# dspcraft/dsc

Hardware: AMD Instinct MI355X
Metric: batched 1-D rfft GSamples/s (higher is better)
Workload: dtype f32

## Files before the change

dsc_amd/csrc/fft_c2c_32k.hip:

```cpp
#define DSC_R2C64K_HELPERS_ONLY 1
#include "fft_r2c_64k.hip"

namespace {

template<bool INV, bool CAST>
__global__ __launch_bounds__(1024) void c2c32k_kernel(const f2 *__restrict__ z, f2 *__restrict__ Z, int batch, const f2 *__restrict__ aux,
                                                      int in_pitch, int in_len) {
    constexpr int EB = CAST ? 4 : 8;
    auto sample = [](__amdgpu_buffer_rsrc_t r, int voff, int soff) {
        if constexpr (CAST) return cf{__builtin_bit_cast(float, __builtin_amdgcn_raw_buffer_load_b32(r, voff, soff, kStream)), 0.0f};
        else return load_c(r, voff, soff);
    };
    extern __shared__ __attribute__((aligned(16))) float lds[];
    float *plane = lds;
    f2 *T = (f2 *) (lds + kPlaneFloats);
    fill_twiddle_table(T, aux);
    const int wave_sgpr = __builtin_amdgcn_readfirstlane(threadIdx.x >> 6);
    constexpr float kScale = 1.0f / (float) kM;

    cf v[32];
    {
        const int row0 = blockIdx.x;
        const __amdgpu_buffer_rsrc_t r0 = __builtin_amdgcn_make_buffer_rsrc(
            (void *) ((const char *) z + (size_t) row0 * in_pitch * EB), 0, row0 < batch ? in_len * EB : 0, 0x00020000);
        const int load_off = thread_id(wave_sgpr) * EB;
#pragma unroll
        for (int a = 0; a < 32; ++a) v[a] = sample(r0, load_off, a * 1024 * EB);
    }
    for (int row = blockIdx.x; row < batch; row += gridDim.x) {
        const int next_row = row + gridDim.x;
        const __amdgpu_buffer_rsrc_t rnext = __builtin_amdgcn_make_buffer_rsrc(
            (void *) ((const char *) z + (size_t) next_row * in_pitch * EB), 0, next_row < batch ? in_len * EB : 0, 0x00020000);
        const __amdgpu_buffer_rsrc_t rout = __builtin_amdgcn_make_buffer_rsrc((void *) (Z + (size_t) row * kM), 0, kM * 8, 0x00020000);
        three_passes<INV>(v, plane, T, aux, wave_sgpr, false, false);
        if (INV) {
#pragma unroll
            for (int p = 0; p < 32; ++p) v[p] = cf{v[p].x * kScale, v[p].y * kScale};
        }
        const int load_off = thread_id(wave_sgpr) * EB;
        staged_time_store(v, plane, rout, wave_sgpr, [&](bool first_half) {
            if (first_half) {
#pragma unroll
                for (int a = 0; a < 16; ++a) v[2 * a] = sample(rnext, load_off, a * 1024 * EB);
            } else {
#pragma unroll
                for (int a = 16; a < 32; ++a) v[2 * (a - 16) + 1] = sample(rnext, load_off, a * 1024 * EB);
            }
        });
        unzip_rows(v);
    }
}

}

void dsc_launch_fft32k_c32(const void *z, void *Z, int batch, int in_pitch, int in_len, bool inverse, bool cast, const void *aux, int n_cu,
                           hipStream_t stream) {
    if (batch <= 0) return;
    static unsigned long long attr_devices = 0;
    if (dsc_first_use_on_device(attr_devices)) {
        DSC_KERNEL_CHECK(hipFuncSetAttribute((const void *) c2c32k_kernel<false, false>, hipFuncAttributeMaxDynamicSharedMemorySize, kLdsBytes));
        DSC_KERNEL_CHECK(hipFuncSetAttribute((const void *) c2c32k_kernel<true, false>, hipFuncAttributeMaxDynamicSharedMemorySize, kLdsBytes));
        DSC_KERNEL_CHECK(hipFuncSetAttribute((const void *) c2c32k_kernel<false, true>, hipFuncAttributeMaxDynamicSharedMemorySize, kLdsBytes));
        DSC_KERNEL_CHECK(hipFuncSetAttribute((const void *) c2c32k_kernel<true, true>, hipFuncAttributeMaxDynamicSharedMemorySize, kLdsBytes));
    }
    const int grid = batch < n_cu ? batch : n_cu;
#define C2C32K(INV, CAST) DSC_LAUNCH((c2c32k_kernel<INV, CAST>), dim3(grid), dim3(1024), kLdsBytes, stream, (const f2 *) z, (f2 *) Z, batch, (const f2 *) aux, in_pitch, in_len)
    if (inverse) { if (cast) C2C32K(true, true); else C2C32K(true, false); }
    else         { if (cast) C2C32K(false, true); else C2C32K(false, false); }
#undef C2C32K
}
```

dsc_amd/csrc/fft_r2c_64k.hip:

```cpp
#include "kernels.h"

#include <hip/hip_runtime.h>

#include <cmath>
#include <cstdlib>
#include <utility>

namespace {

typedef float f2 __attribute__((ext_vector_type(2)));

struct cf { float x, y; };
__device__ __forceinline__ cf operator+(cf a, cf b) { return cf{a.x + b.x, a.y + b.y}; }
__device__ __forceinline__ cf operator-(cf a, cf b) { return cf{a.x - b.x, a.y - b.y}; }
__device__ __forceinline__ cf to_cf(f2 a) { return cf{a.x, a.y}; }
__device__ __forceinline__ f2 to_f2(cf a) { return f2{a.x, a.y}; }

constexpr int kM = 32768;
constexpr int kRowPitch = 34;
constexpr int kPlaneFloats = 1024 * kRowPitch;
constexpr int kLdsBytes = kPlaneFloats * 4 + 1024 * 8;
constexpr int kTabEntries = 1024;

constexpr int kAuxW1024 = 0, kAuxW32768 = 1024, kAuxW65536 = 2048, kAuxEntries = 3072;

__host__ __device__ constexpr int br5(int x) {
    return ((x & 1) << 4) | ((x & 2) << 2) | (x & 4) | ((x & 8) >> 2) | ((x & 16) >> 4);
}

__device__ constexpr float kCos64[17] = {
    1.0f, 0.99518472667219688624f, 0.98078528040323044913f, 0.95694033573220886494f,
    0.92387953251128675613f, 0.88192126434835502971f, 0.83146961230254523708f, 0.77301045336273696081f,
    0.70710678118654752440f, 0.63439328416364549822f, 0.55557023301960222474f, 0.47139673682599764856f,
    0.38268343236508977173f, 0.29028467725446236764f, 0.19509032201612826785f, 0.09801714032956060199f,
    0.0f};

__device__ constexpr float root64_re(int q) {
    q &= 63;
    return q <= 16 ? kCos64[q] : q <= 32 ? -kCos64[32 - q] : q <= 48 ? -kCos64[q - 32] : kCos64[64 - q];
}
__device__ constexpr float root64_im(int q) {
    q &= 63;
    return q <= 16 ? -kCos64[16 - q] : q <= 32 ? -kCos64[q - 16] : q <= 48 ? kCos64[48 - q] : kCos64[q - 48];
}

__device__ __forceinline__ cf cmul(cf a, cf w) {
    return cf{a.x * w.x - a.y * w.y, a.x * w.y + a.y * w.x};
}
__device__ __forceinline__ cf cmul_conj(cf a, cf w) {
    return cf{a.x * w.x + a.y * w.y, a.y * w.x - a.x * w.y};
}

template<bool INV, int M, int K>
__device__ __forceinline__ cf mul_root(cf d) {
    constexpr float c8 = 0.70710678118654752440f;
    if constexpr (K == 0) {
        return d;
    } else if constexpr (4 * K == M) {
        return INV ? cf{-d.y, d.x} : cf{d.y, -d.x};
    } else if constexpr (8 * K == M) {
        return INV ? cf{(d.x - d.y) * c8, (d.x + d.y) * c8} : cf{(d.x + d.y) * c8, (d.y - d.x) * c8};
    } else if constexpr (8 * K == 3 * M) {
        return INV ? cf{-(d.x + d.y) * c8, (d.x - d.y) * c8} : cf{(d.y - d.x) * c8, -(d.x + d.y) * c8};
    } else {
        constexpr float wr = root64_re(K * (64 / M));
        constexpr float wi = INV ? -root64_im(K * (64 / M)) : root64_im(K * (64 / M));
        return cf{d.x * wr - d.y * wi, d.x * wi + d.y * wr};
    }
}

#ifdef DSC_DFT32_DIF
template<bool INV, int M, int G, int... K>
__device__ __forceinline__ void dif_group(cf (&v)[32], std::integer_sequence<int, K...>) {
    (([&] {
         const cf u = v[G + K] + v[G + K + M / 2];
         const cf d = v[G + K] - v[G + K + M / 2];
         v[G + K] = u;
         v[G + K + M / 2] = mul_root<INV, M, K>(d);
     }()),
     ...);
}

template<bool INV, int M, int... G>
__device__ __forceinline__ void dif_stage(cf (&v)[32], std::integer_sequence<int, G...>) {
    (dif_group<INV, M, G * M>(v, std::make_integer_sequence<int, M / 2>{}), ...);
}

template<bool INV>
__device__ __forceinline__ void dft32(cf (&v)[32]) {
    dif_stage<INV, 32>(v, std::make_integer_sequence<int, 1>{});
    dif_stage<INV, 16>(v, std::make_integer_sequence<int, 2>{});
    dif_stage<INV, 8>(v, std::make_integer_sequence<int, 4>{});
    dif_stage<INV, 4>(v, std::make_integer_sequence<int, 8>{});
    dif_stage<INV, 2>(v, std::make_integer_sequence<int, 16>{});
}


#else
constexpr double kCos64d[17] = {
    1.0, 0.99518472667219688624, 0.98078528040323044913, 0.95694033573220886494,
    0.92387953251128675613, 0.88192126434835502971, 0.83146961230254523708, 0.77301045336273696081,
    0.70710678118654752440, 0.63439328416364549822, 0.55557023301960222474, 0.47139673682599764856,
    0.38268343236508977173, 0.29028467725446236764, 0.19509032201612826785, 0.09801714032956060199,
    0.0};

template<bool INV, int E>
__device__ __forceinline__ void dit_butterfly(cf &a, cf &b) {
    if constexpr (E == 0) {
        const cf u = a + b, d = a - b;
        a = u; b = d;
    } else if constexpr (E == 8) {
        const cf u = INV ? cf{a.x - b.y, a.y + b.x} : cf{a.x + b.y, a.y - b.x};
        const cf d = INV ? cf{a.x + b.y, a.y - b.x} : cf{a.x - b.y, a.y + b.x};
        a = u; b = d;
    } else {
        constexpr double c = E <= 8 ? kCos64d[2 * E] : -kCos64d[32 - 2 * E];
        constexpr double sn = (E <= 8 ? kCos64d[16 - 2 * E] : kCos64d[2 * E - 16]);
        constexpr double s = INV ? sn : -sn;
        if constexpr ((c < 0 ? -c : c) >= sn) {
            constexpr float t = (float) (s / c), cc = (float) c;
            float p, q;
            if constexpr (t == 1.0f) { p = b.x - b.y; q = b.y + b.x; }
            else if constexpr (t == -1.0f) { p = b.x + b.y; q = b.y - b.x; }
            else { p = __builtin_fmaf(-t, b.y, b.x); q = __builtin_fmaf(t, b.x, b.y); }
            const cf u = cf{__builtin_fmaf(cc, p, a.x), __builtin_fmaf(cc, q, a.y)};
            const cf d = cf{__builtin_fmaf(-cc, p, a.x), __builtin_fmaf(-cc, q, a.y)};
            a = u; b = d;
        } else {
            constexpr float r = (float) (c / s), ss = (float) s;
            const float pn = __builtin_fmaf(-r, b.x, b.y);
            const float q = __builtin_fmaf(r, b.y, b.x);
            const cf u = cf{__builtin_fmaf(-ss, pn, a.x), __builtin_fmaf(ss, q, a.y)};
            const cf d = cf{__builtin_fmaf(ss, pn, a.x), __builtin_fmaf(-ss, q, a.y)};
            a = u; b = d;
        }
    }
}

constexpr int brev_bits(int x, int bits) {
    int r = 0;
    for (int i = 0; i < bits; ++i) r |= ((x >> i) & 1) << (bits - 1 - i);
    return r;
}

template<bool INV, int S, int G, int... J>
__device__ __forceinline__ void dit_group(cf (&v)[32], std::integer_sequence<int, J...>) {
    constexpr int H = 32 >> S;
    constexpr int E = brev_bits(G, S - 1) * (16 >> (S - 1));
    (dit_butterfly<INV, E>(v[2 * H * G + J], v[2 * H * G + J + H]), ...);
}

template<bool INV, int S, int... G>
__device__ __forceinline__ void dit_stage(cf (&v)[32], std::integer_sequence<int, G...>) {
    (dit_group<INV, S, G>(v, std::make_integer_sequence<int, (32 >> S)>{}), ...);
}

template<bool INV>
__device__ __forceinline__ void dft32(cf (&v)[32]) {
    dit_stage<INV, 1>(v, std::make_integer_sequence<int, 1>{});
    dit_stage<INV, 2>(v, std::make_integer_sequence<int, 2>{});
    dit_stage<INV, 3>(v, std::make_integer_sequence<int, 4>{});
    dit_stage<INV, 4>(v, std::make_integer_sequence<int, 8>{});
    dit_stage<INV, 5>(v, std::make_integer_sequence<int, 16>{});
}
#endif

typedef unsigned int u2 __attribute__((ext_vector_type(2)));
typedef unsigned int u4 __attribute__((ext_vector_type(4)));
typedef float f4 __attribute__((ext_vector_type(4)));

template<int COMP>
__device__ __forceinline__ void plane_write(float *plane, int wbase, const cf (&v)[32]) {
    int wbase_hi = wbase + 16 * (32 * kRowPitch);
    asm("" : "+v"(wbase_hi));
    float *lo16 = plane + wbase;
    float *hi16 = plane + wbase_hi;
#pragma unroll
    for (int p = 0; p < 32; p += 2) lo16[br5(p) * (32 * kRowPitch)] = COMP == 0 ? v[p].x : v[p].y;
#pragma unroll
    for (int p = 1; p < 32; p += 2) hi16[(br5(p) - 16) * (32 * kRowPitch)] = COMP == 0 ? v[p].x : v[p].y;
}

#ifndef DSC_LDS_SPLIT_READS
#define DSC_LDS_SPLIT_READS 1
#endif
__device__ __forceinline__ f2 lds_read_b64(const f2 *p) {
#if DSC_LDS_SPLIT_READS
    return *(const volatile __attribute__((address_space(3))) f2 *) p;
#else
    return *p;
#endif
}

template<int COMP>
__device__ __forceinline__ void plane_read(const float *plane, int row, cf (&v)[32]) {
    const f2 *r = (const f2 *) (plane + __mul24(row, kRowPitch));
#pragma unroll
    for (int m = 0; m < 16; ++m) {
        const f2 t = lds_read_b64(r + m);
        if (COMP == 0) { v[2 * m].x = t.x; v[2 * m + 1].x = t.y; }
        else           { v[2 * m].y = t.x; v[2 * m + 1].y = t.y; }
    }
}

__device__ __forceinline__ void lds_barrier() {
    __builtin_amdgcn_fence(__ATOMIC_RELEASE, "workgroup", "local");
    __builtin_amdgcn_s_barrier();
    __builtin_amdgcn_fence(__ATOMIC_ACQUIRE, "workgroup", "local");
}

__device__ __forceinline__ float bperm(int byte_addr, float x) {
    return __int_as_float(__builtin_amdgcn_ds_bpermute(byte_addr, __float_as_int(x)));
}

__device__ __forceinline__ int column_of(int wave, int lane) {
    int kp = lane < 32 ? 32 * wave + lane : 1024 - 32 * wave - (63 - lane);
    return kp == 1024 ? 512 : kp;
}

#ifdef DSC_R2C64K_PROBE
#define PROBE_ARGS , int io_on
#define PROBE_NULL , 1
#define IO_ON io_on
#else
#define PROBE_ARGS
#define PROBE_NULL
#define IO_ON 1
#endif

__device__ __forceinline__ int thread_id(int wave_sgpr) {
    int zero;
    asm volatile("v_mov_b32 %0, 0" : "=v"(zero));
    const int lane = __builtin_amdgcn_mbcnt_hi(-1, __builtin_amdgcn_mbcnt_lo(-1, zero));
    return (wave_sgpr << 6) | lane;
}

#ifndef DSC_STREAM_AUX
#define DSC_STREAM_AUX 2
#endif
constexpr int kStream = DSC_STREAM_AUX;
__device__ __forceinline__ cf load_c(__amdgpu_buffer_rsrc_t r, int voff, int soff) {
    return to_cf(__builtin_bit_cast(f2, __builtin_amdgcn_raw_buffer_load_b64(r, voff, soff, kStream)));
}
#ifndef DSC_FILTER_EARLY_LOADS
#define DSC_FILTER_EARLY_LOADS 4
#endif
#ifndef DSC_IRFFT_PIN_PASS3
#define DSC_IRFFT_PIN_PASS3 1
#endif
#ifndef DSC_IRFFT_EARLY_PAIRS
#define DSC_IRFFT_EARLY_PAIRS 4
#endif
#ifndef DSC_IRFFT_LOAD_AUX
#define DSC_IRFFT_LOAD_AUX 0
#endif
__device__ __forceinline__ cf load_c_spec(__amdgpu_buffer_rsrc_t r, int voff, int soff) {
    return to_cf(__builtin_bit_cast(f2, __builtin_amdgcn_raw_buffer_load_b64(r, voff, soff, DSC_IRFFT_LOAD_AUX)));
}
__device__ __forceinline__ cf load_c_cached(__amdgpu_buffer_rsrc_t r, int voff, int soff) {
    return to_cf(__builtin_bit_cast(f2, __builtin_amdgcn_raw_buffer_load_b64(r, voff, soff, 0)));
}
template<int POLICY>
__device__ __forceinline__ void store_c(cf a, __amdgpu_buffer_rsrc_t r, int voff, int soff) {
    __builtin_amdgcn_raw_buffer_store_b64(__builtin_bit_cast(u2, to_f2(a)), r, voff, soff, POLICY);
}

__device__ __forceinline__ void fill_twiddle_table(f2 *T, const f2 *aux) {
    const int t = threadIdx.x;
    T[t] = aux[kAuxW1024 + (t >> 5) * (t & 31)];
    __syncthreads();
}

__device__ __forceinline__ void exchange(float *plane, int wbase, int row, const cf (&src)[32], cf (&dst)[32]) {
    plane_write<0>(plane, wbase, src);
    lds_barrier();
    plane_read<0>(plane, row, dst);
    lds_barrier();
    plane_write<1>(plane, wbase, src);
    lds_barrier();
    plane_read<1>(plane, row, dst);
    lds_barrier();
}

struct no_hook { __device__ __forceinline__ void operator()() const {} };

template<bool INV, typename Hook = no_hook>
__device__ __forceinline__ void three_passes(cf (&v)[32], float *plane, const f2 *T, const f2 *aux, int wave_sgpr,
                                             bool mirrored_in, bool mirrored_out, Hook before_pass3 = Hook{}) {
    dft32<INV>(v);
    cf u[32];
    {
        const int t = thread_id(wave_sgpr);
        const int col = mirrored_in ? column_of(t >> 6, t & 63) : t;
        const int hi = col >> 5;
        const f2 *th = T + hi;
#pragma unroll
        for (int r1 = 1; r1 < 32; ++r1) {
            const cf w = to_cf(th[32 * r1]);
            v[br5(r1)] = INV ? cmul_conj(v[br5(r1)], w) : cmul(v[br5(r1)], w);
        }
        exchange(plane, __mul24(col & 31, kRowPitch) + hi, t, v, u);
    }
    dft32<INV>(u);
    {
        const int t = thread_id(wave_sgpr);
        const int hi = t >> 5, lo = t & 31;
        const cf tw2_base = to_cf(aux[kAuxW32768 + __mul24(hi, lo)]);
        u[0] = INV ? cmul_conj(u[0], tw2_base) : cmul(u[0], tw2_base);
        const f2 *tl = T + lo;
#pragma unroll
        for (int r2 = 1; r2 < 32; ++r2) {
            const cf w = cmul(tw2_base, to_cf(tl[32 * r2]));
            u[br5(r2)] = INV ? cmul_conj(u[br5(r2)], w) : cmul(u[br5(r2)], w);
        }
        const int col_out = mirrored_out ? column_of(t >> 6, t & 63) : t;
        exchange(plane, __mul24(hi, kRowPitch) + lo, col_out, u, v);
    }
    before_pass3();
    dft32<INV>(v);
}

__device__ __forceinline__ void real_pair(cf p, cf q, cf wq, float hs, cf &out_k, cf &out_mk) {
    const cf s = cf{p.x + q.x, p.y - q.y};
    const cf d = cf{p.x - q.x, p.y + q.y};
    const cf wd = cmul(d, wq);
    out_k = cf{hs * s.x + wd.x, hs * s.y + wd.y};
    out_mk = cf{hs * s.x - wd.x, wd.y - hs * s.y};
}

__device__ __forceinline__ int partner_byte_addr(int wave, int lane) {
    return ((wave == 0 && (lane == 63 || lane == 0)) ? lane : 63 - lane) * 4;
}

#ifndef DSC_R2C64K_HELPERS_ONLY
__global__ __launch_bounds__(1024) void rfft64k_kernel(const float *__restrict__ x, f2 *__restrict__ X, int batch,
                                                       const f2 *__restrict__ aux, int in_pitch, int in_len PROBE_ARGS) {
    extern __shared__ __attribute__((aligned(16))) float lds[];
    float *plane = lds;
    f2 *T = (f2 *) (lds + kPlaneFloats);
    fill_twiddle_table(T, aux);

    const int wave_sgpr = __builtin_amdgcn_readfirstlane(threadIdx.x >> 6);

    cf v[32];
    {
        const int row0 = blockIdx.x;
        const __amdgpu_buffer_rsrc_t r0 = __builtin_amdgcn_make_buffer_rsrc(
            (void *) (x + (size_t) row0 * in_pitch), 0, row0 < batch ? in_len * 4 * IO_ON : 0, 0x00020000);
        const int load_off = thread_id(wave_sgpr) * 8;
#pragma unroll
        for (int j1 = 0; j1 < 32; ++j1) v[j1] = load_c(r0, load_off, j1 * 8192);
    }

    for (int row = blockIdx.x; row < batch; row += gridDim.x) {
        const int next_row = row + gridDim.x;
        const __amdgpu_buffer_rsrc_t rnext = __builtin_amdgcn_make_buffer_rsrc(
            (void *) (x + (size_t) next_row * in_pitch), 0, next_row < batch ? in_len * 4 * IO_ON : 0, 0x00020000);
        const __amdgpu_buffer_rsrc_t rout =
            __builtin_amdgcn_make_buffer_rsrc((void *) (X + (size_t) row * (kM + 1)), 0, (kM + 1) * 8 * IO_ON, 0x00020000);

        three_passes<false>(v, plane, T, aux, wave_sgpr, false, true);

        const int t4 = thread_id(wave_sgpr);
        const int lane = t4 & 63, wave = t4 >> 6;
        const int kp = column_of(wave, lane);
        const int partner_addr = partner_byte_addr(wave, lane);
        cf xk[16], xm[16];
        const cf zmid = v[br5(16)];
        if (wave_sgpr == 0) {
#pragma unroll
            for (int r = 16; r < 31; ++r) v[br5(r)] = lane == 0 ? v[br5(r + 1)] : v[br5(r)];
            v[br5(31)] = lane == 0 ? v[br5(0)] : v[br5(31)];
        }
#pragma unroll
        for (int k3 = 0; k3 < 16; ++k3) {
            const int src = 31 - br5(k3);
            xm[k3].x = bperm(partner_addr, v[src].x);
            xm[k3].y = bperm(partner_addr, v[src].y);
        }
        {
            const cf wpost = to_cf(aux[kAuxW65536 + kp]);
            const cf post_base = cf{0.5f * wpost.y, -0.5f * wpost.x};
#pragma unroll
            for (int k3 = 0; k3 < 16; ++k3) {
                const cf c = cf{root64_re(k3), root64_im(k3)};
                const cf w = k3 == 0 ? post_base : cmul(post_base, c);
                real_pair(v[br5(k3)], xm[k3], w, 0.5f, xk[k3], xm[k3]);
            }
        }

        f2 *stage = (f2 *) plane;
        const int skew = (int) ((((size_t) (X + (size_t) row * (kM + 1))) >> 3) & 15);
#pragma unroll
        for (int k3 = 0; k3 < 16; ++k3) stage[kp + 1024 * k3] = to_f2(xk[k3]);
        const cf xk15 = xk[15];
        const int load_off = thread_id(wave_sgpr) * 8;
#pragma unroll
        for (int j1 = 0; j1 < 16; ++j1) v[j1] = load_c(rnext, load_off, j1 * 8192);
        lds_barrier();
#pragma unroll
        for (int m = 0; m < 8; ++m) {
            const int k = 2 * (t4 + 1024 * m) - skew;
            if (m > 0 || k >= 0) {
                const f2 lo2 = lds_read_b64(stage + k), hi2 = lds_read_b64(stage + k + 1);
                const f4 q = f4{lo2.x, lo2.y, hi2.x, hi2.y};
                __builtin_amdgcn_raw_buffer_store_b128(__builtin_bit_cast(u4, q), rout, k * 8, 0, kStream);
            } else if (m == 0 && k == -1) {
                __builtin_amdgcn_raw_buffer_store_b64(__builtin_bit_cast(u2, stage[0]), rout, 0, 0, kStream);
            }
            if (m & 1) __builtin_amdgcn_sched_barrier(0);
        }
        lds_barrier();
        constexpr int kStage2 = kM / 2 - 16;
#pragma unroll
        for (int k3 = 0; k3 < 16; ++k3) stage[(kM - kStage2) - kp - 1024 * k3] = to_f2(xm[k3]);
        if (kp >= 1009) stage[kp + 15 * 1024 - kStage2] = to_f2(xk15);
        if (t4 == 0) stage[kM / 2 - kStage2] = f2{zmid.x, -zmid.y};
#pragma unroll
        for (int j1 = 16; j1 < 32; ++j1) v[j1] = load_c(rnext, load_off, j1 * 8192);
        lds_barrier();
#pragma unroll
        for (int m = 0; m < 9; ++m) {
            if (m == 8 && wave != 0) break;
            const int k = kM / 2 + 2 * (t4 + 1024 * m) - skew;
            if (m < 8 || k + 1 <= kM) {
                const f2 lo2 = lds_read_b64(stage + k - kStage2), hi2 = lds_read_b64(stage + k + 1 - kStage2);
                const f4 q = f4{lo2.x, lo2.y, hi2.x, hi2.y};
                __builtin_amdgcn_raw_buffer_store_b128(__builtin_bit_cast(u4, q), rout, k * 8, 0, kStream);
            } else if (m == 8 && k == kM) {
                __builtin_amdgcn_raw_buffer_store_b64(__builtin_bit_cast(u2, stage[k - kStage2]), rout, k * 8, 0, kStream);
            }
            if (m & 1) __builtin_amdgcn_sched_barrier(0);
        }
        lds_barrier();
    }
}

#endif

__device__ __forceinline__ void inverse_prepass_direct(cf (&v)[32], cf y_mid, const f2 *aux, int wave_sgpr) {
    constexpr float kScale = 1.0f / (float) kM;
    const int t1 = thread_id(wave_sgpr);
    const int lane = t1 & 63, wave = t1 >> 6;
    const int c = column_of(wave, lane);
    const int partner_addr = partner_byte_addr(wave, lane);
    if (wave == 0 && lane == 0) { v[0].y = 0.f; v[16].y = 0.f; }
    const cf wpre = to_cf(aux[kAuxW65536 + c]);
    const cf wq_base = cf{0.5f * kScale * wpre.y, 0.5f * kScale * wpre.x};
#pragma unroll
    for (int half = 0; half < 2; ++half) {
        cf zm[8];
#pragma unroll
        for (int i = 0; i < 8; ++i) {
            const int a = half * 8 + i;
            const cf cj = cf{root64_re(a), -root64_im(a)};
            const cf wq = a == 0 ? wq_base : cmul(wq_base, cj);
            real_pair(v[a], v[16 + a], wq, 0.5f * kScale, v[a], zm[i]);
        }
#pragma unroll
        for (int i = 0; i < 8; ++i) {
            const int a = half * 8 + i;
            v[16 + a].x = bperm(partner_addr, zm[i].x);
            v[16 + a].y = bperm(partner_addr, zm[i].y);
        }
    }
    cf w[32];
#pragma unroll
    for (int r = 0; r < 16; ++r) { w[r] = v[r]; w[16 + r] = v[31 - r]; }
    if (wave == 0) {
#pragma unroll
        for (int r = 31; r > 16; --r) w[r] = lane == 0 ? w[r - 1] : w[r];
        w[16] = lane == 0 ? cf{kScale * y_mid.x, -kScale * y_mid.y} : w[16];
    }
#pragma unroll
    for (int r = 0; r < 32; ++r) v[r] = w[r];
}

template<typename IssueNext>
__device__ __forceinline__ void staged_time_store(cf (&v)[32], float *plane, __amdgpu_buffer_rsrc_t rout, int wave_sgpr,
                                                  IssueNext issue_next) {
    f2 *stage = (f2 *) plane;
    const int t4 = thread_id(wave_sgpr);
#pragma unroll
    for (int p = 0; p < 32; p += 2) stage[t4 + 1024 * br5(p)] = to_f2(v[p]);
    issue_next(true);
    lds_barrier();
#pragma unroll
    for (int m = 0; m < 8; ++m) {
        const int k = 2 * (t4 + 1024 * m);
        const f2 lo2 = lds_read_b64(stage + k), hi2 = lds_read_b64(stage + k + 1);
        const f4 q = f4{lo2.x, lo2.y, hi2.x, hi2.y};
        __builtin_amdgcn_raw_buffer_store_b128(__builtin_bit_cast(u4, q), rout, k * 8, 0, kStream);
        if (m & 1) __builtin_amdgcn_sched_barrier(0);
    }
    lds_barrier();
#pragma unroll
    for (int p = 1; p < 32; p += 2) stage[t4 + 1024 * (br5(p) - 16)] = to_f2(v[p]);
    issue_next(false);
    lds_barrier();
#pragma unroll
    for (int m = 0; m < 8; ++m) {
        const int k = 2 * (t4 + 1024 * m);
        const f2 lo2 = lds_read_b64(stage + k), hi2 = lds_read_b64(stage + k + 1);
        const f4 q = f4{lo2.x, lo2.y, hi2.x, hi2.y};
        __builtin_amdgcn_raw_buffer_store_b128(__builtin_bit_cast(u4, q), rout, (kM / 2 + k) * 8, 0, kStream);
        if (m & 1) __builtin_amdgcn_sched_barrier(0);
    }
    lds_barrier();
}

__device__ __forceinline__ void unzip_rows(cf (&v)[32]) {
    cf nxt[32];
#pragma unroll
    for (int a = 0; a < 16; ++a) { nxt[a] = v[2 * a]; nxt[16 + a] = v[2 * a + 1]; }
#pragma unroll
    for (int a = 0; a < 32; ++a) v[a] = nxt[a];
}

#ifndef DSC_R2C64K_HELPERS_ONLY
__global__ __launch_bounds__(1024) void irfft64k_kernel(const f2 *__restrict__ X, float *__restrict__ x, int batch,
                                                        const f2 *__restrict__ aux, int in_pitch, int in_len PROBE_ARGS) {
    extern __shared__ __attribute__((aligned(16))) float lds[];
    float *plane = lds;
    f2 *T = (f2 *) (lds + kPlaneFloats);
    fill_twiddle_table(T, aux);

    const int wave_sgpr = __builtin_amdgcn_readfirstlane(threadIdx.x >> 6);

    cf v[32];
    cf y_mid = cf{0.f, 0.f};
    {
        const int row0 = blockIdx.x;
        const __amdgpu_buffer_rsrc_t r0 = __builtin_amdgcn_make_buffer_rsrc(
            (void *) (X + (size_t) row0 * in_pitch), 0, row0 < batch ? in_len * 8 * IO_ON : 0, 0x00020000);
        const int t0 = thread_id(wave_sgpr);
        const int c = column_of(t0 >> 6, t0 & 63);
        const int pv = (kM - c - 15 * 1024) * 8;
#pragma unroll
        for (int a = 0; a < 16; ++a) {
            v[a] = load_c_spec(r0, c * 8, a * 8192);
            v[16 + a] = load_c_spec(r0, pv, (15 - a) * 8192);
        }
        if (c == 0) y_mid = load_c_spec(r0, (kM / 2) * 8, 0);
    }

    for (int row = blockIdx.x; row < batch; row += gridDim.x) {
        const int next_row = row + gridDim.x;
        const __amdgpu_buffer_rsrc_t rnext = __builtin_amdgcn_make_buffer_rsrc(
            (void *) (X + (size_t) next_row * in_pitch), 0, next_row < batch ? in_len * 8 * IO_ON : 0, 0x00020000);
        const __amdgpu_buffer_rsrc_t rout =
            __builtin_amdgcn_make_buffer_rsrc((void *) (x + (size_t) row * 65536), 0, 65536 * 4 * IO_ON, 0x00020000);

        inverse_prepass_direct(v, y_mid, aux, wave_sgpr);
        constexpr int kEarly = DSC_IRFFT_EARLY_PAIRS;
        cf early[kEarly > 0 ? 2 * kEarly : 1];
        three_passes<true>(v, plane, T, aux, wave_sgpr, true, false, [&]() {
            if constexpr (kEarly > 0) {
                const int t3 = thread_id(wave_sgpr);
                const int c3 = column_of(t3 >> 6, t3 & 63);
                const int pv3 = (kM - c3 - 15 * 1024) * 8;
#pragma unroll
                for (int a = 0; a < kEarly; ++a) {
                    early[2 * a] = load_c_spec(rnext, c3 * 8, a * 8192);
                    early[2 * a + 1] = load_c_spec(rnext, pv3, (15 - a) * 8192);
                }
            }
        });

#if DSC_IRFFT_PIN_PASS3
#pragma unroll
        for (int p = 0; p < 32; p += 8)
            asm volatile("" : "+v"(v[p].x), "+v"(v[p].y), "+v"(v[p + 1].x), "+v"(v[p + 1].y), "+v"(v[p + 2].x), "+v"(v[p + 2].y), "+v"(v[p + 3].x),
                         "+v"(v[p + 3].y), "+v"(v[p + 4].x), "+v"(v[p + 4].y), "+v"(v[p + 5].x), "+v"(v[p + 5].y), "+v"(v[p + 6].x), "+v"(v[p + 6].y),
                         "+v"(v[p + 7].x), "+v"(v[p + 7].y));
#endif
        const int t4 = thread_id(wave_sgpr);
        const int c = column_of(t4 >> 6, t4 & 63);
        const int pv = (kM - c - 15 * 1024) * 8;
        staged_time_store(v, plane, rout, wave_sgpr, [&](bool first_half) {
            if (first_half) {
                y_mid = cf{0.f, 0.f};
                if (c == 0) y_mid = load_c_spec(rnext, (kM / 2) * 8, 0);
#pragma unroll
                for (int i = 0; i < 8; ++i) {
                    v[2 * i] = load_c_spec(rnext, c * 8, (kEarly + i) * 8192);
                    v[16 + 2 * i] = load_c_spec(rnext, pv, (15 - kEarly - i) * 8192);
                }
            } else {
#pragma unroll
                for (int i = 0; i < 8 - kEarly; ++i) {
                    v[2 * i + 1] = load_c_spec(rnext, c * 8, (kEarly + 8 + i) * 8192);
                    v[17 + 2 * i] = load_c_spec(rnext, pv, (7 - kEarly - i) * 8192);
                }
            }
        });
        {
            cf nxt[32];
#pragma unroll
            for (int a = 0; a < 16; ++a) {
                if (a < kEarly)          { nxt[a] = early[2 * a];             nxt[16 + a] = early[2 * a + 1]; }
                else if (a < kEarly + 8) { nxt[a] = v[2 * (a - kEarly)];      nxt[16 + a] = v[16 + 2 * (a - kEarly)]; }
                else                     { nxt[a] = v[2 * (a - kEarly - 8) + 1]; nxt[16 + a] = v[17 + 2 * (a - kEarly - 8)]; }
            }
#pragma unroll
            for (int a = 0; a < 32; ++a) v[a] = nxt[a];
        }
    }
}

__global__ __launch_bounds__(1024) void filter64k_kernel(const float *__restrict__ x, const f2 *__restrict__ H,
                                                         float *__restrict__ y, int batch, const f2 *__restrict__ aux, int in_pitch,
                                                         int in_len) {
    extern __shared__ __attribute__((aligned(16))) float lds[];
    float *plane = lds;
    f2 *T = (f2 *) (lds + kPlaneFloats);
    fill_twiddle_table(T, aux);

    const int wave_sgpr = __builtin_amdgcn_readfirstlane(threadIdx.x >> 6);
    const __amdgpu_buffer_rsrc_t rh = __builtin_amdgcn_make_buffer_rsrc((void *) H, 0, (kM + 1) * 8, 0x00020000);
    constexpr float kScale = 1.0f / (float) kM;

    cf v[32];
    {
        const int row0 = blockIdx.x;
        const __amdgpu_buffer_rsrc_t r0 = __builtin_amdgcn_make_buffer_rsrc(
            (void *) (x + (size_t) row0 * in_pitch), 0, row0 < batch ? in_len * 4 : 0, 0x00020000);
        const int load_off = thread_id(wave_sgpr) * 8;
#pragma unroll
        for (int j1 = 0; j1 < 32; ++j1) v[j1] = load_c(r0, load_off, j1 * 8192);
    }
    for (int row = blockIdx.x; row < batch; row += gridDim.x) {
        const int next_row = row + gridDim.x;
        const __amdgpu_buffer_rsrc_t rnext = __builtin_amdgcn_make_buffer_rsrc(
            (void *) (x + (size_t) next_row * in_pitch), 0, next_row < batch ? in_len * 4 : 0, 0x00020000);
        const __amdgpu_buffer_rsrc_t rout =
            __builtin_amdgcn_make_buffer_rsrc((void *) (y + (size_t) row * 65536), 0, 65536 * 4, 0x00020000);
        three_passes<false>(v, plane, T, aux, wave_sgpr, false, true);

        {
            const int t1 = thread_id(wave_sgpr);
            const int lane = t1 & 63, wave = t1 >> 6;
            const int c = column_of(wave, lane);
            const int partner_addr = partner_byte_addr(wave, lane);
            const cf wc = to_cf(aux[kAuxW65536 + c]);
            const cf post_base = cf{0.5f * wc.y, -0.5f * wc.x};
            const cf pre_base = cf{0.5f * kScale * wc.y, 0.5f * kScale * wc.x};
            if (wave == 0) {
                const cf zmid = v[br5(16)];
                const cf hmid = load_c_cached(rh, (kM / 2) * 8, 0);
                const cf pmid = cmul(cf{zmid.x, -zmid.y}, hmid);
                v[br5(16)] = lane == 0 ? cf{kScale * pmid.x, -kScale * pmid.y} : v[br5(16)];
            }
            cf park = v[br5(16)];
            if (wave == 0) {
#pragma unroll
                for (int r = 16; r < 31; ++r) v[br5(r)] = lane == 0 ? v[br5(r + 1)] : v[br5(r)];
                v[br5(31)] = lane == 0 ? v[br5(0)] : v[br5(31)];
            }
#pragma unroll
            for (int part = 0; part < 8; ++part) {
                cf q[2], zm[2];
#pragma unroll
                for (int i = 0; i < 2; ++i) {
                    const int a = part * 2 + i;
                    q[i].x = bperm(partner_addr, v[br5(31 - a)].x);
                    q[i].y = bperm(partner_addr, v[br5(31 - a)].y);
                }
#pragma unroll
                for (int i = 0; i < 2; ++i) {
                    const int a = part * 2 + i;
                    const cf w64 = cf{root64_re(a), root64_im(a)};
                    cf xk, xm;
                    real_pair(v[br5(a)], q[i], a == 0 ? post_base : cmul(post_base, w64), 0.5f, xk, xm);
                    const cf hk = load_c_cached(rh, c * 8, a * 8192);
                    const cf hm = load_c_cached(rh, (kM - 15 * 1024 - c) * 8, (15 - a) * 8192);
                    cf pk = cmul(xk, hk), pm = cmul(xm, hm);
                    if (a == 0) {
                        pk.y = (c == 0) ? 0.f : pk.y;
                        pm.y = (c == 0) ? 0.f : pm.y;
                    }
                    const cf w64c = cf{root64_re(a), -root64_im(a)};
                    real_pair(pk, pm, a == 0 ? pre_base : cmul(pre_base, w64c), 0.5f * kScale, v[br5(a)], zm[i]);
                }
#pragma unroll
                for (int i = 0; i < 2; ++i) {
                    const int a = part * 2 + i;
                    v[br5(31 - a)].x = bperm(partner_addr, zm[i].x);
                    v[br5(31 - a)].y = bperm(partner_addr, zm[i].y);
                }
                __builtin_amdgcn_sched_barrier(0);
            }
            if (wave == 0) {
#pragma unroll
                for (int r = 31; r > 16; --r) v[br5(r)] = lane == 0 ? v[br5(r - 1)] : v[br5(r)];
                v[br5(16)] = lane == 0 ? park : v[br5(16)];
            }
        }
        cf z[32];
#pragma unroll
        for (int r = 0; r < 32; ++r) z[r] = v[br5(r)];
        constexpr int kEarlyX = DSC_FILTER_EARLY_LOADS;
        cf early[kEarlyX > 0 ? kEarlyX : 1];
        three_passes<true>(z, plane, T, aux, wave_sgpr, true, false, [&]() {
            if constexpr (kEarlyX > 0) {
                const int off = thread_id(wave_sgpr) * 8;
#pragma unroll
                for (int j1 = 0; j1 < kEarlyX; ++j1) early[j1] = load_c(rnext, off, j1 * 8192);
            }
        });
        {
            const int load_off = thread_id(wave_sgpr) * 8;
            staged_time_store(z, plane, rout, wave_sgpr, [&](bool first_half) {
                if (first_half) {
#pragma unroll
                    for (int i = 0; i < 16; ++i) z[2 * i] = load_c(rnext, load_off, (kEarlyX + i) * 8192);
                } else {
#pragma unroll
                    for (int i = 0; i < 16 - kEarlyX; ++i) z[2 * i + 1] = load_c(rnext, load_off, (kEarlyX + 16 + i) * 8192);
                }
            });
#pragma unroll
            for (int j1 = 0; j1 < 32; ++j1) v[j1] = j1 < kEarlyX ? early[j1] : j1 < kEarlyX + 16 ? z[2 * (j1 - kEarlyX)] : z[2 * (j1 - kEarlyX - 16) + 1];
        }
    }
}

#endif

}

#ifndef DSC_R2C64K_HELPERS_ONLY
size_t dsc_r2c64k_table_bytes() { return (size_t) kAuxEntries * sizeof(float) * 2; }

void dsc_r2c64k_build_tables(void *host_dst) {
    float *o = (float *) host_dst;
    auto put = [&](int at, long long k, long long n) {
        const long double a = -2.0L * 3.14159265358979323846264338327950288L * (long double) k / (long double) n;
        o[2 * at] = (float) cosl(a);
        o[2 * at + 1] = (float) sinl(a);
    };
    for (int m = 0; m < kTabEntries; ++m) {
        put(kAuxW1024 + m, m, 1024);
        put(kAuxW32768 + m, m, 32768);
        put(kAuxW65536 + m, m, 65536);
    }
    o[2 * (kAuxW1024 + 256)] = 0.f;  o[2 * (kAuxW1024 + 256) + 1] = -1.f;
    o[2 * (kAuxW1024 + 512)] = -1.f; o[2 * (kAuxW1024 + 512) + 1] = 0.f;
    o[2 * (kAuxW1024 + 768)] = 0.f;  o[2 * (kAuxW1024 + 768) + 1] = 1.f;
}

void dsc_launch_rfft64k(const float *x, void *X, int batch, int in_pitch, int in_len, const void *aux, int n_cu, hipStream_t stream) {
    if (batch <= 0) return;
    static unsigned long long attr_devices = 0;
    if (dsc_first_use_on_device(attr_devices)) {
        DSC_KERNEL_CHECK(hipFuncSetAttribute((const void *) rfft64k_kernel, hipFuncAttributeMaxDynamicSharedMemorySize, kLdsBytes));
    }
    const int grid = batch < n_cu ? batch : n_cu;
    DSC_LAUNCH(rfft64k_kernel, dim3(grid), dim3(1024), kLdsBytes, stream, x, (f2 *) X, batch, (const f2 *) aux, in_pitch, in_len PROBE_NULL);
}

void dsc_launch_irfft64k(const void *X, float *x, int batch, int in_pitch, int in_len, const void *aux, int n_cu, hipStream_t stream) {
    if (batch <= 0) return;
    static unsigned long long attr_devices = 0;
    if (dsc_first_use_on_device(attr_devices)) {
        DSC_KERNEL_CHECK(hipFuncSetAttribute((const void *) irfft64k_kernel, hipFuncAttributeMaxDynamicSharedMemorySize, kLdsBytes));
    }
    const int grid = batch < n_cu ? batch : n_cu;
    DSC_LAUNCH(irfft64k_kernel, dim3(grid), dim3(1024), kLdsBytes, stream, (const f2 *) X, x, batch, (const f2 *) aux, in_pitch, in_len PROBE_NULL);
}
void dsc_launch_filter64k(const float *s, const void *H, float *y, int batch, int in_pitch, int in_len, const void *aux, int n_cu,
                          hipStream_t stream) {
    if (batch <= 0) return;
    static unsigned long long attr_devices = 0;
    if (dsc_first_use_on_device(attr_devices)) {
        DSC_KERNEL_CHECK(hipFuncSetAttribute((const void *) filter64k_kernel, hipFuncAttributeMaxDynamicSharedMemorySize, kLdsBytes));
    }
    const int grid = batch < n_cu ? batch : n_cu;
    DSC_LAUNCH(filter64k_kernel, dim3(grid), dim3(1024), kLdsBytes, stream, s, (const f2 *) H, y, batch, (const f2 *) aux, in_pitch, in_len);
}
#endif
```

Baseline: 660.9.

## Split LDS transpose into quarter steps interleaved with dft32 butterfly stages

Replaces the two-pass split-real/imag plane exchange with a complex (f2) step buffer written in quarters, each written right after its quarter of the radix-32 butterflies and twiddles. Readers are split into two classes so that half of them read after the first two quarters are written, which overlaps LDS traffic with compute and halves the number of exchange round trips. It also remaps thread-to-column assignment (reader_column, spectrum_wave), fuses some twiddle multiplies with FMA, and moves trailing barriers to the start of the store stages. The extra bookkeeping adds register pressure and changes thread-to-data mapping throughout the kernels, which is a correctness risk.

```diff
diff --git a/dsc_amd/csrc/fft_c2c_32k.hip b/dsc_amd/csrc/fft_c2c_32k.hip
--- a/dsc_amd/csrc/fft_c2c_32k.hip
+++ b/dsc_amd/csrc/fft_c2c_32k.hip
@@ -32,7 +32,7 @@
         const __amdgpu_buffer_rsrc_t rnext = __builtin_amdgcn_make_buffer_rsrc(
             (void *) ((const char *) z + (size_t) next_row * in_pitch * EB), 0, next_row < batch ? in_len * EB : 0, 0x00020000);
         const __amdgpu_buffer_rsrc_t rout = __builtin_amdgcn_make_buffer_rsrc((void *) (Z + (size_t) row * kM), 0, kM * 8, 0x00020000);
-        three_passes<INV>(v, plane, T, aux, wave_sgpr, false, false);
+        three_passes<INV>(v, plane, T, aux, wave_sgpr, wave_sgpr, false, false);
         if (INV) {
 #pragma unroll
             for (int p = 0; p < 32; ++p) v[p] = cf{v[p].x * kScale, v[p].y * kScale};
diff --git a/dsc_amd/csrc/fft_r2c_64k.hip b/dsc_amd/csrc/fft_r2c_64k.hip
--- a/dsc_amd/csrc/fft_r2c_64k.hip
+++ b/dsc_amd/csrc/fft_r2c_64k.hip
@@ -17,8 +17,7 @@
 __device__ __forceinline__ f2 to_f2(cf a) { return f2{a.x, a.y}; }
 
 constexpr int kM = 32768;
-constexpr int kRowPitch = 34;
-constexpr int kPlaneFloats = 1024 * kRowPitch;
+constexpr int kPlaneFloats = 1024 * 34;
 constexpr int kLdsBytes = kPlaneFloats * 4 + 1024 * 8;
 constexpr int kTabEntries = 1024;
 
@@ -49,6 +48,12 @@
 }
 __device__ __forceinline__ cf cmul_conj(cf a, cf w) {
     return cf{a.x * w.x + a.y * w.y, a.y * w.x - a.x * w.y};
+}
+
+template<bool INV>
+__device__ __forceinline__ cf twiddle_mul_second_fused(cf a, cf w) {
+    if (INV) return cf{__builtin_fmaf(a.y, w.y, a.x * w.x), __builtin_fmaf(-a.x, w.y, a.y * w.x)};
+    return cf{__builtin_fmaf(-a.y, w.y, a.x * w.x), __builtin_fmaf(a.y, w.x, a.x * w.y)};
 }
 
 template<bool INV, int M, int K>
@@ -95,6 +100,17 @@
     dif_stage<INV, 2>(v, std::make_integer_sequence<int, 16>{});
 }
 
+template<bool INV>
+__device__ __forceinline__ void dft32_head(cf (&v)[32]) {
+    dif_stage<INV, 32>(v, std::make_integer_sequence<int, 1>{});
+    dif_stage<INV, 16>(v, std::make_integer_sequence<int, 2>{});
+}
+template<bool INV, int Q>
+__device__ __forceinline__ void dft32_quarter(cf (&v)[32]) {
+    dif_stage<INV, 8>(v, std::integer_sequence<int, Q>{});
+    dif_stage<INV, 4>(v, std::integer_sequence<int, 2 * Q, 2 * Q + 1>{});
+    dif_stage<INV, 2>(v, std::integer_sequence<int, 4 * Q, 4 * Q + 1, 4 * Q + 2, 4 * Q + 3>{});
+}
 
 #else
 constexpr double kCos64d[17] = {
@@ -163,23 +179,23 @@
     dit_stage<INV, 4>(v, std::make_integer_sequence<int, 8>{});
     dit_stage<INV, 5>(v, std::make_integer_sequence<int, 16>{});
 }
+
+template<bool INV>
+__device__ __forceinline__ void dft32_head(cf (&v)[32]) {
+    dit_stage<INV, 1>(v, std::make_integer_sequence<int, 1>{});
+    dit_stage<INV, 2>(v, std::make_integer_sequence<int, 2>{});
+}
+template<bool INV, int Q>
+__device__ __forceinline__ void dft32_quarter(cf (&v)[32]) {
+    dit_stage<INV, 3>(v, std::integer_sequence<int, Q>{});
+    dit_stage<INV, 4>(v, std::integer_sequence<int, 2 * Q, 2 * Q + 1>{});
+    dit_stage<INV, 5>(v, std::integer_sequence<int, 4 * Q, 4 * Q + 1, 4 * Q + 2, 4 * Q + 3>{});
+}
 #endif
 
 typedef unsigned int u2 __attribute__((ext_vector_type(2)));
 typedef unsigned int u4 __attribute__((ext_vector_type(4)));
 typedef float f4 __attribute__((ext_vector_type(4)));
-
-template<int COMP>
-__device__ __forceinline__ void plane_write(float *plane, int wbase, const cf (&v)[32]) {
-    int wbase_hi = wbase + 16 * (32 * kRowPitch);
-    asm("" : "+v"(wbase_hi));
-    float *lo16 = plane + wbase;
-    float *hi16 = plane + wbase_hi;
-#pragma unroll
-    for (int p = 0; p < 32; p += 2) lo16[br5(p) * (32 * kRowPitch)] = COMP == 0 ? v[p].x : v[p].y;
-#pragma unroll
-    for (int p = 1; p < 32; p += 2) hi16[(br5(p) - 16) * (32 * kRowPitch)] = COMP == 0 ? v[p].x : v[p].y;
-}
 
 #ifndef DSC_LDS_SPLIT_READS
 #define DSC_LDS_SPLIT_READS 1
@@ -190,17 +206,6 @@
 #else
     return *p;
 #endif
-}
-
-template<int COMP>
-__device__ __forceinline__ void plane_read(const float *plane, int row, cf (&v)[32]) {
-    const f2 *r = (const f2 *) (plane + __mul24(row, kRowPitch));
-#pragma unroll
-    for (int m = 0; m < 16; ++m) {
-        const f2 t = lds_read_b64(r + m);
-        if (COMP == 0) { v[2 * m].x = t.x; v[2 * m + 1].x = t.y; }
-        else           { v[2 * m].y = t.x; v[2 * m + 1].y = t.y; }
-    }
 }
 
 __device__ __forceinline__ void lds_barrier() {
@@ -271,50 +276,121 @@
     __syncthreads();
 }
 
-__device__ __forceinline__ void exchange(float *plane, int wbase, int row, const cf (&src)[32], cf (&dst)[32]) {
-    plane_write<0>(plane, wbase, src);
+constexpr int kCPitch = 33;
+static_assert(512 * kCPitch * 8 <= kPlaneFloats * 4, "the step buffer lives inside the plane");
+
+__host__ __device__ constexpr int class_of(int k) { return (k ^ (k >> 1)) & 1; }
+__host__ __device__ constexpr int index_in_class(int k) { return ((k >> 2) << 1) | (k & 1); }
+static_assert(class_of(br5(0)) == 0 && class_of(br5(7)) == 0 && class_of(br5(24)) == 0 && class_of(br5(31)) == 0 &&
+              class_of(br5(8)) == 1 && class_of(br5(23)) == 1, "class 0 = quarters 0 and 3 of a dft32 output");
+
+__device__ __forceinline__ int reader_column(int t) {
+    const int a = t >> 5;
+    return (t & 31) | ((((a >> 3) | ((a & 7) << 2))) << 5);
+}
+__device__ __forceinline__ int spectrum_wave(int wave_sgpr) { return (wave_sgpr >> 2) | ((wave_sgpr & 3) << 2); }
+
+template<int Q>
+__device__ __forceinline__ void quarter_write(f2 *buf, int wbase, const cf (&v)[32]) {
+    int wbase_hi = wbase + 8 * (32 * kCPitch);
+    asm("" : "+v"(wbase_hi));
+    f2 *lo8 = buf + wbase;
+    f2 *hi8 = buf + wbase_hi;
+#pragma unroll
+    for (int p = 8 * Q; p < 8 * Q + 8; ++p)
+        if (index_in_class(br5(p)) < 8) lo8[index_in_class(br5(p)) * (32 * kCPitch)] = to_f2(v[p]);
+#pragma unroll
+    for (int p = 8 * Q; p < 8 * Q + 8; ++p)
+        if (index_in_class(br5(p)) >= 8) hi8[(index_in_class(br5(p)) - 8) * (32 * kCPitch)] = to_f2(v[p]);
+}
+
+__device__ __forceinline__ void step_read(const f2 *buf, int row, cf (&dst)[32]) {
+    const f2 *r = buf + __mul24(row, kCPitch);
+#pragma unroll
+    for (int m = 0; m < 32; ++m) dst[m] = to_cf(lds_read_b64(r + m));
+}
+
+__device__ __forceinline__ void pin(cf (&v)[32]) {
+#pragma unroll
+    for (int p = 0; p < 32; p += 8)
+        asm volatile("" : "+v"(v[p].x), "+v"(v[p].y), "+v"(v[p + 1].x), "+v"(v[p + 1].y), "+v"(v[p + 2].x), "+v"(v[p + 2].y), "+v"(v[p + 3].x),
+                     "+v"(v[p + 3].y), "+v"(v[p + 4].x), "+v"(v[p + 4].y), "+v"(v[p + 5].x), "+v"(v[p + 5].y), "+v"(v[p + 6].x), "+v"(v[p + 6].y),
+                     "+v"(v[p + 7].x), "+v"(v[p + 7].y));
+}
+
+template<typename Finish>
+__device__ __forceinline__ void exchange(f2 *buf, int wbase, int rclass, int rrow, cf (&src)[32], cf (&dst)[32], Finish finish) {
+    pin(src);
     lds_barrier();
-    plane_read<0>(plane, row, dst);
+    finish(std::integral_constant<int, 0>{});
+    quarter_write<0>(buf, wbase, src);
+    finish(std::integral_constant<int, 3>{});
+    quarter_write<3>(buf, wbase, src);
     lds_barrier();
-    plane_write<1>(plane, wbase, src);
+    cf r[32];
+    if (rclass == 0) step_read(buf, rrow, r);
+    finish(std::integral_constant<int, 1>{});
     lds_barrier();
-    plane_read<1>(plane, row, dst);
+    quarter_write<1>(buf, wbase, src);
+    finish(std::integral_constant<int, 2>{});
+    quarter_write<2>(buf, wbase, src);
     lds_barrier();
+    if (rclass != 0) step_read(buf, rrow, r);
+#pragma unroll
+    for (int m = 0; m < 32; ++m) dst[m] = r[m];
 }
 
 struct no_hook { __device__ __forceinline__ void operator()() const {} };
 
 template<bool INV, typename Hook = no_hook>
-__device__ __forceinline__ void three_passes(cf (&v)[32], float *plane, const f2 *T, const f2 *aux, int wave_sgpr,
+__device__ __forceinline__ void three_passes(cf (&v)[32], float *plane, const f2 *T, const f2 *aux, int wave_sgpr, int col_wave,
                                              bool mirrored_in, bool mirrored_out, Hook before_pass3 = Hook{}) {
-    dft32<INV>(v);
+    f2 *buf = (f2 *) plane;
+    const int wave_class = ((wave_sgpr >> 2) ^ (wave_sgpr >> 3)) & 1;
+    dft32_head<INV>(v);
     cf u[32];
     {
         const int t = thread_id(wave_sgpr);
-        const int col = mirrored_in ? column_of(t >> 6, t & 63) : t;
+        const int col = mirrored_in ? column_of(col_wave, t & 63) : t;
         const int hi = col >> 5;
         const f2 *th = T + hi;
-#pragma unroll
-        for (int r1 = 1; r1 < 32; ++r1) {
-            const cf w = to_cf(th[32 * r1]);
-            v[br5(r1)] = INV ? cmul_conj(v[br5(r1)], w) : cmul(v[br5(r1)], w);
-        }
-        exchange(plane, __mul24(col & 31, kRowPitch) + hi, t, v, u);
-    }
-    dft32<INV>(u);
+        const int rc = reader_column(t);
+        exchange(buf, __mul24(col & 31, kCPitch) + hi, wave_class, (index_in_class(rc >> 5) << 5) | (rc & 31), v, u, [&](auto Q) {
+            constexpr int kQ = decltype(Q)::value;
+            dft32_quarter<INV, kQ>(v);
+#pragma unroll
+            for (int p = 8 * kQ; p < 8 * kQ + 8; ++p) {
+                if (p == 0) continue;
+                const cf w = to_cf(th[32 * br5(p)]);
+                v[p] = INV ? cmul_conj(v[p], w) : cmul(v[p], w);
+            }
+        });
+    }
+    dft32_head<INV>(u);
     {
         const int t = thread_id(wave_sgpr);
-        const int hi = t >> 5, lo = t & 31;
+        const int rc = reader_column(t);
+        const int hi = rc >> 5, lo = rc & 31;
         const cf tw2_base = to_cf(aux[kAuxW32768 + __mul24(hi, lo)]);
-        u[0] = INV ? cmul_conj(u[0], tw2_base) : cmul(u[0], tw2_base);
         const f2 *tl = T + lo;
-#pragma unroll
-        for (int r2 = 1; r2 < 32; ++r2) {
-            const cf w = cmul(tw2_base, to_cf(tl[32 * r2]));
-            u[br5(r2)] = INV ? cmul_conj(u[br5(r2)], w) : cmul(u[br5(r2)], w);
-        }
-        const int col_out = mirrored_out ? column_of(t >> 6, t & 63) : t;
-        exchange(plane, __mul24(hi, kRowPitch) + lo, col_out, u, v);
+        const int col_out = mirrored_out ? column_of(col_wave, t & 63) : rc;
+        const int k2 = col_out >> 5;
+        const int rclass = mirrored_out ? class_of(k2) : wave_class;
+        exchange(buf, __mul24(hi, kCPitch) + lo, rclass, (index_in_class(k2) << 5) | (col_out & 31), u, v, [&](auto Q) {
+            constexpr int kQ = decltype(Q)::value;
+            dft32_quarter<INV, kQ>(u);
+#ifdef DSC_DFT32_DIF
+            constexpr bool kSumsOnly = false;
+#else
+            constexpr bool kSumsOnly = true;
+#endif
+#pragma unroll
+            for (int p = 8 * kQ; p < 8 * kQ + 8; ++p) {
+                const cf w = p == 0 ? tw2_base : cmul(tw2_base, to_cf(tl[32 * br5(p)]));
+                if (kSumsOnly && p < 4) u[p] = twiddle_mul_second_fused<INV>(u[p], w);
+                else u[p] = INV ? cmul_conj(u[p], w) : cmul(u[p], w);
+            }
+        });
     }
     before_pass3();
     dft32<INV>(v);
@@ -359,15 +435,16 @@
         const __amdgpu_buffer_rsrc_t rout =
             __builtin_amdgcn_make_buffer_rsrc((void *) (X + (size_t) row * (kM + 1)), 0, (kM + 1) * 8 * IO_ON, 0x00020000);
 
-        three_passes<false>(v, plane, T, aux, wave_sgpr, false, true);
+        const int cw = spectrum_wave(wave_sgpr);
+        three_passes<false>(v, plane, T, aux, wave_sgpr, cw, false, true);
 
         const int t4 = thread_id(wave_sgpr);
         const int lane = t4 & 63, wave = t4 >> 6;
-        const int kp = column_of(wave, lane);
-        const int partner_addr = partner_byte_addr(wave, lane);
+        const int kp = column_of(cw, lane);
+        const int partner_addr = partner_byte_addr(cw, lane);
         cf xk[16], xm[16];
         const cf zmid = v[br5(16)];
-        if (wave_sgpr == 0) {
+        if (cw == 0) {
 #pragma unroll
             for (int r = 16; r < 31; ++r) v[br5(r)] = lane == 0 ? v[br5(r + 1)] : v[br5(r)];
             v[br5(31)] = lane == 0 ? v[br5(0)] : v[br5(31)];
@@ -391,6 +468,7 @@
 
         f2 *stage = (f2 *) plane;
         const int skew = (int) ((((size_t) (X + (size_t) row * (kM + 1))) >> 3) & 15);
+        lds_barrier();
 #pragma unroll
         for (int k3 = 0; k3 < 16; ++k3) stage[kp + 1024 * k3] = to_f2(xk[k3]);
         const cf xk15 = xk[15];
@@ -432,7 +510,6 @@
             }
             if (m & 1) __builtin_amdgcn_sched_barrier(0);
         }
-        lds_barrier();
     }
 }
 
@@ -481,8 +558,10 @@
                                                   IssueNext issue_next) {
     f2 *stage = (f2 *) plane;
     const int t4 = thread_id(wave_sgpr);
-#pragma unroll
-    for (int p = 0; p < 32; p += 2) stage[t4 + 1024 * br5(p)] = to_f2(v[p]);
+    const int c4 = reader_column(t4);
+    lds_barrier();
+#pragma unroll
+    for (int p = 0; p < 32; p += 2) stage[c4 + 1024 * br5(p)] = to_f2(v[p]);
     issue_next(true);
     lds_barrier();
 #pragma unroll
@@ -495,7 +574,7 @@
     }
     lds_barrier();
 #pragma unroll
-    for (int p = 1; p < 32; p += 2) stage[t4 + 1024 * (br5(p) - 16)] = to_f2(v[p]);
+    for (int p = 1; p < 32; p += 2) stage[c4 + 1024 * (br5(p) - 16)] = to_f2(v[p]);
     issue_next(false);
     lds_barrier();
 #pragma unroll
@@ -506,7 +585,6 @@
         __builtin_amdgcn_raw_buffer_store_b128(__builtin_bit_cast(u4, q), rout, (kM / 2 + k) * 8, 0, kStream);
         if (m & 1) __builtin_amdgcn_sched_barrier(0);
     }
-    lds_barrier();
 }
 
 __device__ __forceinline__ void unzip_rows(cf (&v)[32]) {
@@ -554,7 +632,7 @@
         inverse_prepass_direct(v, y_mid, aux, wave_sgpr);
         constexpr int kEarly = DSC_IRFFT_EARLY_PAIRS;
         cf early[kEarly > 0 ? 2 * kEarly : 1];
-        three_passes<true>(v, plane, T, aux, wave_sgpr, true, false, [&]() {
+        three_passes<true>(v, plane, T, aux, wave_sgpr, wave_sgpr, true, false, [&]() {
             if constexpr (kEarly > 0) {
                 const int t3 = thread_id(wave_sgpr);
                 const int c3 = column_of(t3 >> 6, t3 & 63);
@@ -635,11 +713,12 @@
             (void *) (x + (size_t) next_row * in_pitch), 0, next_row < batch ? in_len * 4 : 0, 0x00020000);
         const __amdgpu_buffer_rsrc_t rout =
             __builtin_amdgcn_make_buffer_rsrc((void *) (y + (size_t) row * 65536), 0, 65536 * 4, 0x00020000);
-        three_passes<false>(v, plane, T, aux, wave_sgpr, false, true);
+        const int cw = spectrum_wave(wave_sgpr);
+        three_passes<false>(v, plane, T, aux, wave_sgpr, cw, false, true);
 
         {
             const int t1 = thread_id(wave_sgpr);
-            const int lane = t1 & 63, wave = t1 >> 6;
+            const int lane = t1 & 63, wave = cw;
             const int c = column_of(wave, lane);
             const int partner_addr = partner_byte_addr(wave, lane);
             const cf wc = to_cf(aux[kAuxW65536 + c]);
@@ -701,7 +780,7 @@
         for (int r = 0; r < 32; ++r) z[r] = v[br5(r)];
         constexpr int kEarlyX = DSC_FILTER_EARLY_LOADS;
         cf early[kEarlyX > 0 ? kEarlyX : 1];
-        three_passes<true>(z, plane, T, aux, wave_sgpr, true, false, [&]() {
+        three_passes<true>(z, plane, T, aux, wave_sgpr, cw, true, false, [&]() {
             if constexpr (kEarlyX > 0) {
                 const int off = thread_id(wave_sgpr) * 8;
 #pragma unroll
```

New measurement: 674.1 (median of 6 runs). 1.02x the previous value.
